# amathislab/HOISDF

Hardware: AMD Instinct MI355X
Metric: samples/sec (img + 2048 SDF queries) fwd+bwd at 1/2/4/8 MI355X (higher is better)
Workload: dtype f32 (emulated contractions, f32 accumulate, f16x2 form: operands as scaled hi + lo f16 pieces x 3 products - 22 operand bits, one power-of-two scale per ROW of a linear layer's row operand, per (sample, head) of the attention operands, per weight matrix; the attention backward's dS as three pieces x

## Files before the change

hoisdf_amd/csrc/chain.h:

```cpp
#pragma once
#include <stdlib.h>

#include <mutex>
#include <unordered_map>

#include "common.h"

namespace hoisdf {
namespace {

constexpr long EMU_MIN_ROWS = 2048;
constexpr long EMU_DW_MIN_ROWS = 8192;

inline bool al16(const void* p) { return (reinterpret_cast<uintptr_t>(p) & 15) == 0; }

struct SavedMags {
  std::mutex mu;
  std::unordered_map<const void*, int> on;
  void put(const void* key, bool v) { if (!key) return; std::lock_guard<std::mutex> l(mu); if (on.size() > 8192) on.clear(); on[key] = v ? 1 : 0; }
  int get(const void* key) { std::lock_guard<std::mutex> l(mu); auto it = on.find(key); return it == on.end() ? -1 : it->second; }
};
inline SavedMags& saved_mags() { static SavedMags s; return s; }

struct Ctx {
  hipStream_t st; void* stream;
  Bump* ws;
  bool dry;
  bool emu;
  int rc = HOISDF_OK;
  bool ok() const { return rc == HOISDF_OK; }
};

inline bool emu_small(const Ctx& c, long M, const float* a, long lda, const float* W, long ldw, int N, int K) {
  if (!c.emu || M > hoisdf_linear_emu_small_max_rows() || N % 4 || K % 4 || lda % 4 || ldw % 4) return false;
  return c.dry || hoisdf_linear_emu_small_supported(a, lda, W, ldw, M, N, K);
}
bool emu_rows(const Ctx& c, long M, const float* a, long lda, int contraction) {
  return c.emu && M >= EMU_MIN_ROWS && contraction % 4 == 0 && lda % 4 == 0 && (c.dry || al16(a));
}
const void* image_of(Ctx& c, const void* given, const float* W, int ldw, int N, int K, int transpose) {
  if (given) return given;
  void* img = c.ws->take(hoisdf_linear_emu_image_bytes(transpose ? K : N, transpose ? N : K));
  if (c.dry) return nullptr;
  if (!img) { c.rc = HOISDF_ERR_WORKSPACE; return nullptr; }
  c.rc = hoisdf_linear_emu_prepare(W, ldw, N, K, transpose, img, c.stream);
  return img;
}
void lin_fwd(Ctx& c, const float* x, int ldx, const float* W, int ldw, const void* img, const float* b, float* y, int ldy, long M, int N,
             int K, int act, float p, uint64_t seed, uint32_t* bits, int K_pad = 0, const uint32_t* x_mag = nullptr, uint32_t* y_mag = nullptr,
             uint32_t* y_heads = nullptr, int head_L = 0) {
  if (!c.ok()) return;
  if (K_pad < K || (K_pad + 15) / 16 != (K + 15) / 16) K_pad = K;
  if (emu_rows(c, M, x, ldx, K_pad)) {
    const void* im = image_of(c, img, W, ldw, N, K, 0);
    if (c.dry || !c.ok()) return;
    c.rc = linear_fwd_emu_mag(x, ldx, im, b, y, ldy, M, N, K_pad, act, p, seed, bits, x_mag, y_mag, c.stream, y_heads, head_L);
    return;
  }
  if (c.dry) return;
  if (emu_small(c, M, x, ldx, W, ldw, N, K)) { c.rc = hoisdf_linear_fwd_emu_small(x, ldx, W, ldw, b, y, ldy, M, N, K, act, p, seed, bits, c.stream); return; }
  c.rc = hoisdf_linear_fwd(x, ldx, W, ldw, b, y, ldy, M, N, K, act, p, seed, bits, c.stream);
}
void lin_bwd_input(Ctx& c, const float* dy, int lddy, const uint32_t* bits, float p, const float* W, int ldw, const void* img_t, float* dx,
                   int lddx, long M, int N, int K, int accumulate, const uint32_t* dy_mag = nullptr, uint32_t* dx_mag = nullptr,
                   uint32_t* dx_heads = nullptr, int head_L = 0) {
  if (!c.ok()) return;
  if (!bits) p = 0.f;
  if (emu_rows(c, M, dy, lddy, N)) {
    const void* im = image_of(c, img_t, W, ldw, N, K, 1);
    if (c.dry || !c.ok()) return;
    c.rc = linear_bwd_input_emu_mag(dy, lddy, bits, p, im, dx, lddx, M, N, K, accumulate, dy_mag, accumulate ? nullptr : dx_mag, c.stream,
                                    accumulate ? nullptr : dx_heads, head_L);
    return;
  }
  if (c.dry) return;
  if (emu_small(c, M, dy, lddy, W, ldw, N, K)) { c.rc = hoisdf_linear_bwd_input_emu_small(dy, lddy, bits, p, W, ldw, dx, lddx, M, N, K, accumulate, c.stream); return; }
  c.rc = hoisdf_linear_bwd_input(dy, lddy, bits, p, W, ldw, dx, lddx, M, N, K, accumulate, c.stream);
}
void lin_bwd_weight(Ctx& c, const float* dy, int lddy, const uint32_t* bits, float p, const float* x, int ldx, float* dW, float* db, long M,
                    int N, int K, int K_pad = 0, const uint32_t* dy_mag = nullptr, const uint32_t* x_mag = nullptr) {
  if (!c.ok()) return;
  if (!bits) p = 0.f;
  if (K_pad < K) K_pad = K;
  const bool emu = c.emu && M >= EMU_DW_MIN_ROWS && (N < K ? N : K) >= 64 && N % 4 == 0 && K_pad % 4 == 0 && lddy % 4 == 0 && ldx % 4 == 0 &&
                   (c.dry || (al16(dy) && al16(x) && al16(dW)));
  if (emu) {
    const long nws = hoisdf_linear_bwd_weight_emu_workspace(M, N, K_pad);
    float* w = c.ws->floats(nws > 4 ? nws : 4);
    if (!c.dry) {
      if (!w) { c.rc = HOISDF_ERR_WORKSPACE; return; }
      if (dy_mag || x_mag) c.rc = linear_bwd_weight_emu_mag(dy, lddy, bits, p, x, ldx, dW, K_pad, db, M, N, K_pad, w, nws, dy_mag, x_mag, c.stream);
      else c.rc = hoisdf_linear_bwd_weight_emu(dy, lddy, bits, p, x, ldx, dW, K_pad, db, M, N, K_pad, w, nws, c.stream);
    }
    return;
  }
  if (c.emu && M <= hoisdf_linear_emu_small_max_rows()) {
    if (!c.dry) c.rc = hoisdf_linear_bwd_weight_emu_small(dy, lddy, bits, p, x, ldx, dW, K_pad, db, M, N, K_pad, c.stream);
    return;
  }
  long nws = 0; float* w = nullptr;
  if (deterministic_mode()) {
    nws = hoisdf_linear_bwd_weight_workspace(M, N, K_pad);
    if (nws > 0) w = c.ws->floats(nws);
    if (!c.dry && nws > 0 && !w) { c.rc = HOISDF_ERR_WORKSPACE; return; }
  }
  if (c.dry) return;
  c.rc = hoisdf_linear_bwd_weight(dy, lddy, bits, p, x, ldx, dW, K_pad, db, M, N, K_pad, w, nws, c.stream);
}


}
}
```

hoisdf_amd/csrc/heads.hip:

```cpp
#include "chain.h"

using namespace hoisdf;

namespace {
constexpr int MLP_MAX = HOISDF_MLP_MAX_LAYERS;
inline long bits_words(int N) { return (N + 31) / 32; }

struct MlpSaved { float* h[MLP_MAX]; uint32_t* bits[MLP_MAX]; uint32_t* mag; };

bool mlp_ok(const hoisdf_mlp* m) {
  if (!m || m->n_layers < 1 || m->n_layers > MLP_MAX) return false;
  for (int i = 0; i <= m->n_layers; ++i) if (m->dims[i] <= 0) return false;
  return true;
}
void mlp_carve(const hoisdf_mlp* m, long M, Bump& b, MlpSaved& s) {
  const int last = m->n_layers - 1;
  for (int i = 0; i < m->n_layers; ++i) {
    s.h[i] = i < last ? b.floats(M * m->dims[i + 1]) : nullptr;
    const bool act = i < last || m->act_last;
    s.bits[i] = act ? static_cast<uint32_t*>(b.take(M * bits_words(m->dims[i + 1]) * 4)) : nullptr;
  }
  s.mag = static_cast<uint32_t*>(b.take((long)m->n_layers * M * 4));
}
inline bool chain_mags_on(const Ctx& c, long M) { return c.emu && emu_form_h2() && M >= EMU_MIN_ROWS; }
uint32_t* chain_mags(Ctx& c, long M, int n) {
  if (!chain_mags_on(c, M)) return nullptr;
  uint32_t* p = static_cast<uint32_t*>(c.ws->take((long)n * M * 4));
  if (c.dry || !p || !c.ok()) return nullptr;
  if (hipMemsetAsync(p, 0, (size_t)n * M * 4, c.st) != hipSuccess) { c.rc = HOISDF_ERR_LAUNCH; return nullptr; }
  return p;
}
void mlp_forward(Ctx& c, const hoisdf_mlp* m, const float* x, int ldx, long M, const MlpSaved& s, float* y, int ldy, const uint32_t* x_mag = nullptr) {
  const int last = m->n_layers - 1;
  const float* in = x; int ldin = ldx;
  uint32_t* mg = chain_mags_on(c, M) && !c.dry && s.mag && c.ok() ? s.mag : nullptr;
  if (!c.dry) saved_mags().put(s.mag, mg != nullptr);
  if (mg && hipMemsetAsync(mg, 0, (size_t)m->n_layers * M * 4, c.st) != hipSuccess) { c.rc = HOISDF_ERR_LAUNCH; return; }
  const uint32_t* in_mag = mg ? x_mag : nullptr;
  if (mg && !in_mag && emu_rows(c, M, x, ldx, m->dims[0])) {
    if ((c.rc = emu_mag_measure(x, ldx, M, m->dims[0], mg, c.st)) != HOISDF_OK) return;
    in_mag = mg;
  }
  for (int i = 0; i < m->n_layers; ++i) {
    float* out = i < last ? s.h[i] : y;
    const int ldo = i < last ? m->dims[i + 1] : ldy;
    uint32_t* out_mag = mg && i < last && emu_rows(c, M, in, ldin, m->dims[i]) ? mg + (long)(i + 1) * M : nullptr;
    lin_fwd(c, in, ldin, m->w[i], m->dims[i], m->img[i], m->b[i], out, ldo, M, m->dims[i + 1], m->dims[i], s.bits[i] ? 1 : 0, 0.f, 0, s.bits[i], 0,
            in_mag, out_mag);
    in = out; ldin = ldo; in_mag = out_mag;
  }
}
void mlp_backward(Ctx& c, const hoisdf_mlp* m, const hoisdf_mlp_grads* G, const float* x, int ldx, long M, const MlpSaved& s, const float* dy,
                  int lddy, float* dx, int lddx, int accumulate_dx, const uint32_t* x_mag = nullptr) {
  const float* g = dy; int ldg = lddy;
  const int last = m->n_layers - 1;
  uint32_t* mg = chain_mags(c, M, m->n_layers + 1);
  const bool fwd_mags = mg && s.mag && saved_mags().get(s.mag) != 0;
  const uint32_t* g_mag = nullptr;
  if (mg && emu_rows(c, M, dy, lddy, m->dims[last + 1])) {
    if ((c.rc = emu_mag_measure(dy, lddy, M, m->dims[last + 1], mg + (long)(last + 1) * M, c.st)) != HOISDF_OK) return;
    g_mag = mg + (long)(last + 1) * M;
  }
  for (int i = last; i >= 0; --i) {
    const float* in = i > 0 ? s.h[i - 1] : x;
    const int ldin = i > 0 ? m->dims[i] : ldx;
    const uint32_t* in_mag = !fwd_mags ? nullptr : i > 0 ? (emu_rows(c, M, i > 1 ? s.h[i - 2] : x, i > 1 ? m->dims[i - 1] : ldx, m->dims[i - 1]) ? s.mag + (long)i * M : nullptr)
                                                         : (x_mag ? x_mag : (emu_rows(c, M, x, ldx, m->dims[0]) ? s.mag : nullptr));
    lin_bwd_weight(c, g, ldg, s.bits[i], 0.f, in, ldin, G->dw[i], G->db[i], M, m->dims[i + 1], m->dims[i], 0, g_mag, g_mag ? in_mag : nullptr);
    if (i == 0 && !dx) break;
    float* gin = i > 0 ? c.ws->floats(M * m->dims[i]) : dx;
    const int ldgin = i > 0 ? m->dims[i] : lddx;
    if (!c.dry && c.ok() && !gin) { c.rc = HOISDF_ERR_WORKSPACE; return; }
    uint32_t* gin_mag = mg && i > 0 && emu_rows(c, M, g, ldg, m->dims[i + 1]) ? mg + (long)i * M : nullptr;
    lin_bwd_input(c, g, ldg, s.bits[i], 0.f, m->w[i], m->dims[i], m->img_t[i], gin, ldgin, M, m->dims[i + 1], m->dims[i], i == 0 ? accumulate_dx : 0,
                  g_mag, gin_mag);
    g = gin; ldg = ldgin; g_mag = gin_mag;
  }
}
const uint32_t* enc_mag(const Ctx& c, const hoisdf_mlp* m, const float* x, int ldx, long M, const MlpSaved& s) {
  return chain_mags_on(c, M) && !c.dry && s.mag && saved_mags().get(s.mag) != 0 && emu_rows(c, M, x, ldx, m->dims[0]) ? s.mag : nullptr;
}
bool grads_ok(const hoisdf_mlp* m, const hoisdf_mlp_grads* G) {
  if (!G) return false;
  for (int i = 0; i < m->n_layers; ++i) if (!G->dw[i] || !G->db[i]) return false;
  return true;
}

struct TokSaved { float* feat; float* fea; MlpSaved mlp; };
void tok_carve(const hoisdf_mlp* m, long M, bool own_feat, Bump& b, TokSaved& s) {
  s.feat = own_feat ? b.floats(M * m->dims[0]) : nullptr;
  s.fea = b.floats(M * m->dims[m->n_layers]);
  mlp_carve(m, M, b, s.mlp);
}

struct VoteSaved { float *off, *cls, *stats; MlpSaved vote, cl; };
void vote_carve(const hoisdf_mlp* mv, const hoisdf_mlp* mc, long M, int LB, int J, Bump& b, VoteSaved& s) {
  s.off = b.floats(M * 3 * J); s.cls = b.floats(M * J); s.stats = b.floats((long)LB * J * 2);
  mlp_carve(mv, M, b, s.vote); mlp_carve(mc, M, b, s.cl);
}
}

extern "C" long hoisdf_tokens_saved_bytes(const hoisdf_mlp* mlp, long n_rows, int gather_inside) {
  if (!mlp_ok(mlp) || n_rows <= 0) return 0;
  Bump b(nullptr, 0); TokSaved s;
  tok_carve(mlp, n_rows, gather_inside != 0, b, s);
  return b.off + 256;
}

static int tokens_backward(const hoisdf_mlp* mlp, const hoisdf_mlp_grads* G, const float* feat, long M, TokSaved& s, const float* dtok,
                           const float* sdf, const float* beta, float* dfeat, int accumulate_dfeat, float* dbeta, int B, int P, int S, int row0,
                           int D, Bump& ws, bool dry, void* stream) {
  Ctx c{as_stream(stream), stream, &ws, dry, gemm_emu_mode()};
  const int F = mlp->dims[mlp->n_layers];
  float* dfea = ws.floats(M * F);
  float* part = ws.floats(hoisdf_token_build_bwd_partials());
  if (!dry) {
    if (!dfea || !part) { set_error("tokens_bwd: workspace too small"); return HOISDF_ERR_WORKSPACE; }
    c.rc = hoisdf_token_build_bwd_ordered(dtok, s.fea, F, sdf, beta, dfea, F, dbeta, part, B, P, S, row0, D, stream);
  }
  mlp_backward(c, mlp, G, feat, mlp->dims[0], M, s.mlp, dfea, F, dfeat, mlp->dims[0], accumulate_dfeat);
  if (c.ok() && !dry && ws.overflow) { set_error("tokens_bwd: workspace too small"); return HOISDF_ERR_WORKSPACE; }
  return c.rc;
}

extern "C" long hoisdf_tokens_workspace_bytes(const hoisdf_mlp* mlp, long n_rows, int backward_pass) {
  if (!mlp_ok(mlp) || n_rows <= 0) return 0;
  Bump ws(nullptr, 0), sv(nullptr, 0);
  TokSaved s; tok_carve(mlp, n_rows, false, sv, s);
  Ctx c{nullptr, nullptr, &ws, true, gemm_emu_mode()};
  if (backward_pass) {
    hoisdf_mlp_grads G{};
    (void)tokens_backward(mlp, &G, nullptr, n_rows, s, nullptr, nullptr, nullptr, reinterpret_cast<float*>(1), 0, nullptr, 1, 1, 1, 0, 1, ws, true, nullptr);
  } else {
    mlp_forward(c, mlp, nullptr, mlp->dims[0], n_rows, s.mlp, nullptr, mlp->dims[mlp->n_layers]);
  }
  return ws.off + 256;
}

extern "C" int hoisdf_tokens_fwd(const hoisdf_pyramid* pyr, const float* points, const float* center, const float* cam_intr, float scale,
                                 int img_h, int img_w, const float* feat_in, const float* cam_in, const hoisdf_mlp* mlp, const float* pe,
                                 const float* sdf, const float* beta_ptr, float* tok, float* fea_out, float* cam_out, int B, int P, int S,
                                 int row0, int D, void* saved, long saved_bytes, void* workspace, long workspace_bytes, void* stream) {
  HOISDF_REQUIRE(mlp_ok(mlp) && center && pe && sdf && beta_ptr && tok && saved && workspace, HOISDF_ERR_INVALID, "tokens_fwd: null pointer / bad MLP");
  HOISDF_REQUIRE(B > 0 && P > 0 && S >= row0 + P && row0 >= 0 && mlp->act_last && mlp->dims[mlp->n_layers] == D - 33, HOISDF_ERR_INVALID,
                 "tokens_fwd: bad sizes (the MLP must end in D - 33 = %d activated columns)", D - 33);
  const bool gather = feat_in == nullptr;
  HOISDF_REQUIRE(gather ? (pyr && points && cam_intr && cam_out) : (cam_in != nullptr), HOISDF_ERR_INVALID,
                 "tokens_fwd: either gathered rows + their camera points, or a pyramid + points + cam_out");
  const long M = (long)B * P;
  HOISDF_REQUIRE(saved_bytes >= hoisdf_tokens_saved_bytes(mlp, M, gather), HOISDF_ERR_WORKSPACE, "tokens_fwd: saved buffer of %ld bytes, need %ld", saved_bytes,
                 hoisdf_tokens_saved_bytes(mlp, M, gather));
// ... 9 lines not shown
  }
  mlp_forward(c, mlp, feat, C, M, s.mlp, s.fea, F);
  if (c.ok()) c.rc = hoisdf_token_build_fwd(cam, center, pe, s.fea, F, sdf, beta_ptr, tok, B, P, S, row0, D, stream);
  if (c.ok() && fea_out && hipMemcpyAsync(fea_out, s.fea, sizeof(float) * M * F, hipMemcpyDeviceToDevice, c.st) != hipSuccess) c.rc = HOISDF_ERR_LAUNCH;
  if (c.ok() && (sv.overflow || ws.overflow)) c.rc = HOISDF_ERR_WORKSPACE;
  if (c.rc == HOISDF_ERR_WORKSPACE) set_error("tokens_fwd: workspace (%ld bytes) too small", workspace_bytes);
  return c.rc;
}

extern "C" int hoisdf_tokens_bwd(const hoisdf_pyramid_grad* dpyr, const float* points, const float* center, const float* cam_intr, float scale,
                                 int img_h, int img_w, const float* feat_in, const hoisdf_mlp* mlp, const float* sdf, const float* beta_ptr,
                                 const float* dtok, const void* saved, long saved_bytes, const hoisdf_mlp_grads* grads, float* dfeat,
                                 int accumulate_dfeat, float* dbeta, int B, int P, int S, int row0, int D, void* workspace, long workspace_bytes,
                                 void* stream) {
  HOISDF_REQUIRE(mlp_ok(mlp) && grads_ok(mlp, grads) && sdf && beta_ptr && dtok && saved && dbeta && workspace, HOISDF_ERR_INVALID,
                 "tokens_bwd: null pointer (every weight-gradient buffer is required, zero-filled)");
  const bool gather = feat_in == nullptr;
  const long M = (long)B * P;
  HOISDF_REQUIRE(B > 0 && P > 0 && saved_bytes >= hoisdf_tokens_saved_bytes(mlp, M, gather), HOISDF_ERR_INVALID, "tokens_bwd: bad sizes / saved buffer");
  HOISDF_REQUIRE(gather ? (points && center && cam_intr) : true, HOISDF_ERR_INVALID, "tokens_bwd: the gather's arguments are needed again");
  Bump sv(const_cast<void*>(saved), saved_bytes), ws(workspace, workspace_bytes);
  TokSaved s; tok_carve(mlp, M, gather, sv, s);
  const int C = mlp->dims[0];
  float* df = dfeat;
  int acc = accumulate_dfeat;
  if (gather && dpyr && !df) {
    df = ws.floats(M * C); acc = 0;
    if (!df) { set_error("tokens_bwd: workspace too small"); return HOISDF_ERR_WORKSPACE; }
  }
  int rc = tokens_backward(mlp, grads, gather ? s.feat : feat_in, M, s, dtok, sdf, beta_ptr, df, acc, dbeta, B, P, S, row0, D, ws, false, stream);
  if (rc == HOISDF_OK && gather && dpyr && df)
    rc = hoisdf_project_gather_bwd(dpyr, points, nullptr, M, P, center, cam_intr, scale, img_h, img_w, df, C, stream);
  return rc;
}

extern "C" long hoisdf_heads_vote_saved_bytes(const hoisdf_mlp* vote, const hoisdf_mlp* cls, int L, int B, int P, int J) {
  if (!mlp_ok(vote) || !mlp_ok(cls) || L <= 0 || B <= 0 || P <= 0 || J <= 0) return 0;
  Bump b(nullptr, 0); VoteSaved s;
  vote_carve(vote, cls, (long)L * B * P, L * B, J, b, s);
  return b.off + 256;
}

static int heads_vote_backward(const hoisdf_mlp* mv, const hoisdf_mlp* mc, const hoisdf_mlp_grads* Gv, const hoisdf_mlp_grads* Gc, const float* enc,
                               const float* pts, const float* gt, float radius, const float* joints, VoteSaved& s, const float* djoints,
                               const float* dl3d, const float* dbce, float* denc, int L, int B, int P, int J, Bump& ws, bool dry, void* stream) {
  Ctx c{as_stream(stream), stream, &ws, dry, gemm_emu_mode()};
  const long M = (long)L * B * P;
  float* doff = ws.floats(M * 3 * J); float* dcls = ws.floats(M * J);
  if (!dry) {
    if (!doff || !dcls) { set_error("heads_vote_bwd: workspace too small"); return HOISDF_ERR_WORKSPACE; }
    c.rc = hoisdf_vote_loss_bwd(s.off, s.cls, pts, gt, radius, joints, s.stats, djoints, dl3d, dbce, doff, dcls, L, B, P, J, stream);
  }
  const int E = mv->dims[0];
  mlp_backward(c, mv, Gv, enc, E, M, s.vote, doff, 3 * J, denc, E, 0);
  mlp_backward(c, mc, Gc, enc, E, M, s.cl, dcls, J, denc, E, 1, enc_mag(c, mv, enc, E, M, s.vote));
  if (c.ok() && !dry && ws.overflow) { set_error("heads_vote_bwd: workspace too small"); return HOISDF_ERR_WORKSPACE; }
  return c.rc;
}

extern "C" long hoisdf_heads_vote_workspace_bytes(const hoisdf_mlp* vote, const hoisdf_mlp* cls, int L, int B, int P, int J, int backward_pass) {
  if (!mlp_ok(vote) || !mlp_ok(cls) || L <= 0 || B <= 0 || P <= 0 || J <= 0) return 0;
  const long M = (long)L * B * P;
  Bump ws(nullptr, 0), sv(nullptr, 0);
  VoteSaved s; vote_carve(vote, cls, M, L * B, J, sv, s);
  if (backward_pass) {
    hoisdf_mlp_grads G{};
    (void)heads_vote_backward(vote, cls, &G, &G, nullptr, nullptr, nullptr, 0.f, nullptr, s, nullptr, nullptr, nullptr, reinterpret_cast<float*>(1), L, B, P, J, ws,
                              true, nullptr);
  } else {
    Ctx c{nullptr, nullptr, &ws, true, gemm_emu_mode()};
    mlp_forward(c, vote, nullptr, vote->dims[0], M, s.vote, nullptr, 3 * J);
    mlp_forward(c, cls, nullptr, cls->dims[0], M, s.cl, nullptr, J);
  }
  return ws.off + 256;
}

extern "C" int hoisdf_heads_vote_fwd(const float* enc, const hoisdf_mlp* vote, const hoisdf_mlp* cls, const float* pts, const float* joint_gt_mm,
                                     float radius, float* joints, float* l3d_sum, float* bce_sum, float* near_sum, int L, int B, int P, int J,
                                     void* saved, long saved_bytes, void* workspace, long workspace_bytes, void* stream) {
  HOISDF_REQUIRE(enc && mlp_ok(vote) && mlp_ok(cls) && pts && joint_gt_mm && joints && l3d_sum && bce_sum && near_sum && saved && workspace,
                 HOISDF_ERR_INVALID, "heads_vote_fwd: null pointer / bad MLP");
  HOISDF_REQUIRE(L > 0 && B > 0 && P > 0 && J > 0 && vote->dims[vote->n_layers] == 3 * J && cls->dims[cls->n_layers] == J &&
                     vote->dims[0] == cls->dims[0] && !vote->act_last && !cls->act_last,
                 HOISDF_ERR_INVALID, "heads_vote_fwd: the vote MLP must end in 3 J = %d, the class MLP in J = %d plain columns", 3 * J, J);
  HOISDF_REQUIRE(saved_bytes >= hoisdf_heads_vote_saved_bytes(vote, cls, L, B, P, J), HOISDF_ERR_WORKSPACE, "heads_vote_fwd: saved buffer too small");
  const long M = (long)L * B * P;
  Bump sv(saved, saved_bytes), ws(workspace, workspace_bytes);
  VoteSaved s; vote_carve(vote, cls, M, L * B, J, sv, s);
  Ctx c{as_stream(stream), stream, &ws, false, gemm_emu_mode()};
  const int E = vote->dims[0];
  mlp_forward(c, vote, enc, E, M, s.vote, s.off, 3 * J);
  mlp_forward(c, cls, enc, E, M, s.cl, s.cls, J, enc_mag(c, vote, enc, E, M, s.vote));
  if (c.ok()) c.rc = hoisdf_vote_loss_fwd(s.off, s.cls, pts, joint_gt_mm, radius, joints, s.stats, l3d_sum, bce_sum, near_sum, L, B, P, J, stream);
  if (c.ok() && (sv.overflow || ws.overflow)) c.rc = HOISDF_ERR_WORKSPACE;
  if (c.rc == HOISDF_ERR_WORKSPACE) set_error("heads_vote_fwd: workspace (%ld bytes) too small", workspace_bytes);
  return c.rc;
}

extern "C" int hoisdf_heads_vote_bwd(const float* enc, const hoisdf_mlp* vote, const hoisdf_mlp* cls, const float* pts, const float* joint_gt_mm,
                                     float radius, const float* joints, const void* saved, long saved_bytes, const float* djoints,
                                     const float* dl3d_sum, const float* dbce_sum, const hoisdf_mlp_grads* vote_grads,
                                     const hoisdf_mlp_grads* cls_grads, float* denc, int L, int B, int P, int J, void* workspace,
                                     long workspace_bytes, void* stream) {
  HOISDF_REQUIRE(enc && mlp_ok(vote) && mlp_ok(cls) && grads_ok(vote, vote_grads) && grads_ok(cls, cls_grads) && pts && joint_gt_mm && joints && saved &&
                     denc && workspace,
                 HOISDF_ERR_INVALID, "heads_vote_bwd: null pointer (every weight-gradient buffer is required, zero-filled)");
  HOISDF_REQUIRE(L > 0 && B > 0 && P > 0 && J > 0 && saved_bytes >= hoisdf_heads_vote_saved_bytes(vote, cls, L, B, P, J), HOISDF_ERR_INVALID,
                 "heads_vote_bwd: bad sizes / saved buffer");
  Bump sv(const_cast<void*>(saved), saved_bytes), ws(workspace, workspace_bytes);
  VoteSaved s; vote_carve(vote, cls, (long)L * B * P, L * B, J, sv, s);
  return heads_vote_backward(vote, cls, vote_grads, cls_grads, enc, pts, joint_gt_mm, radius, joints, s, djoints, dl3d_sum, dbce_sum, denc, L, B, P, J, ws, false,
                             stream);
}
```

hoisdf_amd/csrc/sdf_query.hip:

```cpp
#include "common.h"

using namespace hoisdf;

namespace {
constexpr int HID0 = 512, LAT = 256, PF = 33, H1 = 223, X0 = LAT + PF, CAT_K = 516, X0_COL = 224;
constexpr int CAT_LD = 544;
inline long align64(long v) { return (v + 63) / 64 * 64; }
constexpr long EMU_MIN_ROWS_Q = 2048;

inline long emu_scratch_bytes(int C) {
  const long a = hoisdf_linear_emu_image_bytes(HID0, C), b = hoisdf_linear_emu_image_bytes(HID0, CAT_K);
  return ((a > b ? a : b) + 255) / 256 * 256;
}

int layer(const float* x, int ldx, const float* W, int ldw, const float* b, float* y, int ldy, long M, int N, int K,
          int K_pad, float drop_p, uint64_t seed, void* emu_img, const void* given, void* stream, const uint32_t* x_mag = nullptr,
          uint32_t* y_mag = nullptr, bool* y_has = nullptr) {
  if (y_has) *y_has = false;
  if (emu_img && M >= EMU_MIN_ROWS_Q && hoisdf_linear_emu_supported(x, ldx, K_pad) && (K_pad + 15) / 16 == (K + 15) / 16) {
    if (!given) { if (int rc = hoisdf_linear_emu_prepare(W, ldw, N, K, 0, emu_img, stream)) return rc; }
    if (y_has) *y_has = y_mag != nullptr;
    return linear_fwd_emu_mag(x, ldx, given ? given : emu_img, b, y, ldy, M, N, K_pad, 1, drop_p, seed, nullptr, x_mag, y_mag, stream);
  }
  return hoisdf_linear_fwd(x, ldx, W, ldw, b, y, ldy, M, N, K, 1, drop_p, seed, nullptr, stream);
// ... 157 lines not shown
  int rc = hoisdf_lattice_fill(center, cam_intr, bbox, scale, bins_n, B, offsets, pts, sidx, lidx, stream);
  if (rc) return rc;
  rc = hoisdf_sdf_query_fwd(pyr, pts, sidx, n, 1, center, cam_intr, scale, img_h, img_w, nullptr, nullptr, w, clamp, drop_p, seed, sdf, raw, pe,
                            nullptr, qws, qbytes, stream);
  if (rc) return rc;
  rc = hoisdf_select_smallest_abs(raw, offsets, counts_device, B, num_points, sel, stream);
  if (rc) return rc;
  const long ns = (long)B * num_points;
  rc = hoisdf_gather_rows(pts, 3, sel, ns, 3, points_out, 3, stream);
  if (rc) return rc;
  rc = hoisdf_gather_rows(sdf, 1, sel, ns, 1, sdf_out, 1, stream);
  if (rc) return rc;
  if (pe_out) rc = hoisdf_gather_rows(pe, 30, sel, ns, 30, pe_out, 30, stream);
  return rc;
}

#include "chain.h"

namespace {
struct TrainSaved { float *feat, *ha, *cat, *h0, *h2, *h3, *raw; uint32_t *ba, *bf, *b0, *b1, *b2, *b3; uint32_t* mag; };
enum { TM_FEAT = 0, TM_HA = 1, TM_CAT = 2, TM_H0 = 3, TM_H2 = 4, TM_N = 5 };
inline bool train_mags(const Ctx& c, long n) { return c.emu && emu_form_h2() && n >= EMU_MIN_ROWS; }
inline long bits_words(int N) { return (N + 31) / 32; }
void train_carve(long n, int C, Bump& b, TrainSaved& s) {
  s.feat = b.floats(n * C); s.ha = b.floats(n * HID0); s.cat = b.floats(n * CAT_LD); s.h0 = b.floats(n * HID0); s.h2 = b.floats(n * HID0);
  s.h3 = b.floats(n * HID0); s.raw = b.floats(n);
  s.ba = static_cast<uint32_t*>(b.take(n * bits_words(HID0) * 4)); s.bf = static_cast<uint32_t*>(b.take(n * bits_words(LAT) * 4));
  s.b0 = static_cast<uint32_t*>(b.take(n * bits_words(HID0) * 4)); s.b1 = static_cast<uint32_t*>(b.take(n * bits_words(H1 + 1) * 4));
  s.b2 = static_cast<uint32_t*>(b.take(n * bits_words(HID0) * 4)); s.b3 = static_cast<uint32_t*>(b.take(n * bits_words(HID0) * 4));
  s.mag = static_cast<uint32_t*>(b.take((long)TM_N * n * 4));
}
}

extern "C" long hoisdf_sdf_query_train_saved_bytes(long n_rows, int C) {
  if (n_rows <= 0 || C <= 0) return 0;
  Bump b(nullptr, 0); TrainSaved s;
  train_carve(n_rows, C, b, s);
  return b.off + 256;
}

static int sdf_train_forward(const hoisdf_pyramid* pyr, const float* points, const int32_t* sample_idx, long n, int rps, const float* center,
                             const float* cam_intr, float scale, int img_h, int img_w, const hoisdf_sdf_weights* w, float clamp, float drop_p,
                             uint64_t seed, float* sdf, float* pe, float* cam_out, Bump& saved, Bump& ws, bool dry, void* stream) {
  Ctx c{as_stream(stream), stream, &ws, dry, gemm_emu_mode()};
  TrainSaved s;
  const int C = w ? w->C : 1;
  train_carve(n, C, saved, s);
  const bool mags = train_mags(c, n) && !dry && s.mag;
  if (!dry) saved_mags().put(s.mag, mags);
  auto mg = [&](int i) -> uint32_t* { return mags ? s.mag + (long)i * n : nullptr; };
  if (!dry) {
    if (mags) c.rc = hipMemsetAsync(s.mag, 0, (size_t)TM_N * n * 4, c.st) == hipSuccess ? HOISDF_OK : HOISDF_ERR_LAUNCH;
    if (c.ok()) c.rc = project_gather_fwd_mag(pyr, points, sample_idx, n, rps, center, cam_intr, scale, img_h, img_w, s.feat, C, cam_out, nullptr, mg(TM_FEAT), stream);
    if (c.ok()) c.rc = hipMemsetAsync(s.cat, 0, sizeof(float) * n * CAT_LD, c.st) == hipSuccess ? HOISDF_OK : HOISDF_ERR_LAUNCH;
  }
  float* x0 = dry ? nullptr : s.cat + X0_COL;
  lin_fwd(c, s.feat, C, w->sdfin_w0, C, w->emu_img[0], w->sdfin_b0, s.ha, HID0, n, HID0, C, 1, 0.f, 0, s.ba, 0, mg(TM_FEAT), mg(TM_HA));
  lin_fwd(c, s.ha, HID0, w->sdfin_w1, HID0, w->emu_img[1], w->sdfin_b1, x0, CAT_LD, n, LAT, HID0, 1, 0.f, 0, s.bf, 0, mg(TM_HA), mg(TM_CAT));
  if (!dry && c.ok()) c.rc = posenc_fwd_mag(points, n, s.cat, CAT_LD, X0_COL + LAT, pe, mg(TM_CAT), stream);
  lin_fwd(c, x0, CAT_LD, w->dec_w0, w->dec_ld0, w->emu_img[2], w->dec_b0, s.h0, HID0, n, HID0, X0, 1, drop_p, seed, s.b0, X0 + 3, mg(TM_CAT), mg(TM_H0));
  lin_fwd(c, s.h0, HID0, w->dec_w1, HID0, w->emu_img[3], w->dec_b1, s.cat, CAT_LD, n, H1 + 1, HID0, 1, drop_p, seed + 1, s.b1, 0, mg(TM_H0), mg(TM_CAT));
  lin_fwd(c, s.cat, CAT_LD, w->dec_w2, CAT_K, w->emu_img[4], w->dec_b2, s.h2, HID0, n, HID0, CAT_K, 1, drop_p, seed + 2, s.b2, 0, mg(TM_CAT), mg(TM_H2));
  lin_fwd(c, s.h2, HID0, w->dec_w3, HID0, w->emu_img[5], w->dec_b3, s.h3, HID0, n, HID0, HID0, 1, drop_p, seed + 3, s.b3, 0, mg(TM_H2), nullptr);
  if (!dry && c.ok()) c.rc = hoisdf_sdf_head_fwd(s.h3, HID0, w->dec_w4, w->dec_b4, s.raw, sdf, n, HID0, clamp, stream);
  return c.rc;
}

static int sdf_train_backward(const hoisdf_pyramid_grad* dpyr, const float* points, const int32_t* sample_idx, long n, int rps, const float* center,
                              const float* cam_intr, float scale, int img_h, int img_w, const hoisdf_sdf_weights* w, float clamp, float drop_p,
                              const float* d_sdf, const hoisdf_sdf_weight_grads* G, Bump& saved, Bump& ws, bool dry, void* stream) {
  Ctx c{as_stream(stream), stream, &ws, dry, gemm_emu_mode()};
  TrainSaved s;
  const int C = w ? w->C : 1;
  train_carve(n, C, saved, s);
  float* dh3 = ws.floats(n * HID0); float* dh2 = ws.floats(n * HID0); float* dcat = ws.floats(n * CAT_LD); float* dh0 = ws.floats(n * HID0);
  float* dha = ws.floats(n * HID0); float* dfeat = ws.floats(n * (long)C);
  if (!dry && (!dh3 || !dh2 || !dcat || !dh0 || !dha || !dfeat)) { set_error("sdf_query_bwd: workspace too small"); return HOISDF_ERR_WORKSPACE; }
  enum { BM_DH3 = 0, BM_DH2 = 1, BM_DCAT = 2, BM_DH0 = 3, BM_DHA = 4, BM_N = 5 };
  uint32_t* bmag = static_cast<uint32_t*>(ws.take((long)BM_N * n * 4));
  const bool mags = train_mags(c, n) && !dry && bmag && s.mag;
  const bool fmags = mags && saved_mags().get(s.mag) != 0;
  auto mg = [&](int i) -> uint32_t* { return mags ? bmag + (long)i * n : nullptr; };
  auto fm = [&](int i) -> const uint32_t* { return fmags ? s.mag + (long)i * n : nullptr; };
  if (mags) c.rc = hipMemsetAsync(bmag, 0, (size_t)BM_N * n * 4, c.st) == hipSuccess ? HOISDF_OK : HOISDF_ERR_LAUNCH;
  if (!dry && c.ok()) c.rc = sdf_head_bwd_mag(d_sdf, s.raw, s.h3, HID0, w->dec_w4, dh3, HID0, G->d_dec_w4, G->d_dec_b4, n, HID0, clamp, mg(BM_DH3), stream);
  lin_bwd_input(c, dh3, HID0, s.b3, drop_p, w->dec_w3, HID0, w->emu_img_t[5], dh2, HID0, n, HID0, HID0, 0, mg(BM_DH3), mg(BM_DH2));
  lin_bwd_weight(c, dh3, HID0, s.b3, drop_p, s.h2, HID0, G->d_dec_w3, G->d_dec_b3, n, HID0, HID0, 0, mg(BM_DH3), fm(TM_H2));
  lin_bwd_input(c, dh2, HID0, s.b2, drop_p, w->dec_w2, CAT_K, w->emu_img_t[4], dcat, CAT_LD, n, HID0, CAT_K, 0, mg(BM_DH2), mg(BM_DCAT));
  lin_bwd_weight(c, dh2, HID0, s.b2, drop_p, s.cat, CAT_LD, G->d_dec_w2, G->d_dec_b2, n, HID0, CAT_K, 0, mg(BM_DH2), fm(TM_CAT));
  lin_bwd_input(c, dcat, CAT_LD, s.b1, drop_p, w->dec_w1, HID0, w->emu_img_t[3], dh0, HID0, n, H1 + 1, HID0, 0, mg(BM_DCAT), mg(BM_DH0));
  lin_bwd_weight(c, dcat, CAT_LD, s.b1, drop_p, s.h0, HID0, G->d_dec_w1, G->d_dec_b1, n, H1 + 1, HID0, 0, mg(BM_DCAT), fm(TM_H0));
  float* dx0 = dry ? nullptr : dcat + X0_COL;
  const float* x0 = dry ? nullptr : s.cat + X0_COL;
  lin_bwd_input(c, dh0, HID0, s.b0, drop_p, w->dec_w0, w->dec_ld0, w->emu_img_t[2], dx0, CAT_LD, n, HID0, X0, 1, mg(BM_DH0), nullptr);
  lin_bwd_weight(c, dh0, HID0, s.b0, drop_p, x0, CAT_LD, G->d_dec_w0, G->d_dec_b0, n, HID0, X0, X0 + 3, mg(BM_DH0), fm(TM_CAT));
  lin_bwd_input(c, dx0, CAT_LD, s.bf, 0.f, w->sdfin_w1, HID0, w->emu_img_t[1], dha, HID0, n, LAT, HID0, 0, nullptr, mg(BM_DHA));
  lin_bwd_weight(c, dx0, CAT_LD, s.bf, 0.f, s.ha, HID0, G->d_sdfin_w1, G->d_sdfin_b1, n, LAT, HID0, 0, nullptr, fm(TM_HA));
  lin_bwd_input(c, dha, HID0, s.ba, 0.f, w->sdfin_w0, C, w->emu_img_t[0], dfeat, C, n, HID0, C, 0, mg(BM_DHA), nullptr);
  lin_bwd_weight(c, dha, HID0, s.ba, 0.f, s.feat, C, G->d_sdfin_w0, G->d_sdfin_b0, n, HID0, C, 0, mg(BM_DHA), fm(TM_FEAT));
  if (!dry && c.ok() && dpyr)
    c.rc = hoisdf_project_gather_bwd(dpyr, points, sample_idx, n, rps, center, cam_intr, scale, img_h, img_w, dfeat, C, stream);
  if (c.ok() && !dry && ws.overflow) { set_error("sdf_query_bwd: workspace too small"); return HOISDF_ERR_WORKSPACE; }
  return c.rc;
}

extern "C" long hoisdf_sdf_query_train_workspace_bytes(long n_rows, int C, int backward_pass) {
  if (n_rows <= 0 || C <= 0) return 0;
// ... 42 lines not shown
```

hoisdf_amd/ops.py:

```python
from __future__ import annotations

import ctypes as C
import math
import os
from typing import Optional, Sequence

import numpy as np
import torch

from . import _lib
from ._lib import (MLP_MAX_LAYERS, DecoderLayerDesc, DecoderLayerGrads, DecoderLayerWeights, EncoderLayerDesc,
                   EncoderLayerGrads, EncoderLayerWeights, Mlp, MlpGrads, PoseOutputs, Pyramid, SdfWeightGrads, SdfWeights, call, lib)
from .emu_images import WeightImageCache, prepare_batch_table

_SEED = [0x9E3779B97F4A7C15, 0]
_WEIGHT_GEN = [0]


def deterministic() -> bool:
    return bool(lib().hoisdf_get_deterministic())


def set_deterministic(on: bool) -> None:
    lib().hoisdf_set_deterministic(int(bool(on)))
# ... 184 lines not shown
        return (None, *out)


class _ProjectGather(torch.autograd.Function):
    @staticmethod
    def forward(ctx, points, sample_idx, center, cam_intr, scale, img_hw, acc, *levels):
        ctx.acc = acc
        pyr = PyramidNHWC(levels)
        pts = points.reshape(-1, 3).contiguous()
        _chk(pts, center, cam_intr)
        n = pts.shape[0]
        rps = points.shape[-2] if sample_idx is None else 1
        feat = torch.empty(n, pyr.C, device=pts.device, dtype=torch.float32)
        cam = torch.empty(n, 3, device=pts.device, dtype=torch.float32)
        s = pyr.struct()
        call("hoisdf_project_gather_fwd", C.byref(s), _p(pts), _p(sample_idx), n, rps, _p(center), _p(cam_intr),
             float(scale), img_hw[0], img_hw[1], _p(feat), pyr.C, _p(cam), None, _st())
        ctx.save_for_backward(pts, sample_idx, center, cam_intr)
        ctx.meta = (float(scale), img_hw, rps, [tuple(l.shape) for l in pyr.levels], pyr.B)
        ctx.mark_non_differentiable(cam)
        return feat, cam

    @staticmethod
    def backward(ctx, dfeat, _dcam):
        pts, sample_idx, center, cam_intr = ctx.saved_tensors
        scale, img_hw, rps, shapes, B = ctx.meta
        dfeat = dfeat.contiguous()
        acc = ctx.acc
        if acc is not None:
            grads = acc.bufs
            acc.flat.record_stream(torch.cuda.current_stream(dfeat.device))
        else:
            grads = [torch.zeros(sh, device=dfeat.device, dtype=torch.float32) for sh in shapes]
        g = _pyramid_struct(grads, B)
        call("hoisdf_project_gather_bwd", C.byref(g), _p(pts), _p(sample_idx), pts.shape[0], rps, _p(center),
             _p(cam_intr), scale, img_hw[0], img_hw[1], _p(dfeat), dfeat.shape[1], _st())
        if acc is not None:
            ev = torch.cuda.Event()
            ev.record(torch.cuda.current_stream(dfeat.device))
            acc.events.append(ev)
            acc.touched = True
            return (None,) * (7 + len(shapes))
        return (None, None, None, None, None, None, None, *grads)


def project_gather(pyr: PyramidNHWC, points, center, cam_intr, scale, img_hw=(256, 256), sample_idx=None):
    return _ProjectGather.apply(points, sample_idx, center.contiguous(), cam_intr.contiguous(), scale,
                                tuple(img_hw), pyr.acc, *pyr.levels)


_GEMM_EMU = os.environ.get("HOISDF_GEMM", "emu") != "f32"
_GEMM_EMU_MIN_ROWS = 2048
_GEMM_EMU_DW_MIN_ROWS = 8192
_GEMM_EMU_DW_MIN_WIDTH = 64
_EMU_CACHE = WeightImageCache()


def set_gemm_emu(on: bool) -> None:
    global _GEMM_EMU
    _GEMM_EMU = bool(on)
    lib().hoisdf_set_gemm_emu(int(_GEMM_EMU))


def gemm_emu() -> bool:
    return _GEMM_EMU


_EMU_SMALL_MAX = [None]


def _emu_small_max_rows() -> int:
    if _EMU_SMALL_MAX[0] is None:
        _EMU_SMALL_MAX[0] = lib().hoisdf_linear_emu_small_max_rows()
    return _EMU_SMALL_MAX[0]


def _emu_small_ok(M: int, a: torch.Tensor, lda: int, W: torch.Tensor, N: int, K: int) -> bool:
    if not _GEMM_EMU:
        return False
    return (1 <= M <= _emu_small_max_rows() and N % 4 == 0 and K % 4 == 0 and lda % 4 == 0 and W.stride(0) % 4 == 0
            and a.data_ptr() % 16 == 0 and W.data_ptr() % 16 == 0)


def _emu_ok(M: int, a: torch.Tensor, lda: int, contraction: int) -> bool:
    return (_GEMM_EMU and M >= _GEMM_EMU_MIN_ROWS and contraction % 4 == 0 and lda % 4 == 0
            and a.data_ptr() % 16 == 0)


def _emu_image(W: torch.Tensor, transpose: bool) -> torch.Tensor:
    return _EMU_CACHE.get(W, transpose, _WEIGHT_GEN[0])


_H2 = [None]


def _h2() -> bool:
    if _H2[0] is None:
        _H2[0] = lib().hoisdf_linear_emu_pieces() == 2
    return _H2[0]


def _mag_measure(a2, lda, M, K):
    if not _h2():
        return None
    words = torch.empty(max(int(M), 1), device=a2.device, dtype=torch.int32)
    call("hoisdf_mag_measure", _p(a2), lda, M, K, _p(words), _st())
    a2._hoisdf_words = (words, a2._version, a2.data_ptr(), lda, M, K)
    return words


def _head_measure(a2, lda, M, groups, L):
    nb = (M + L - 1) // L
    words = torch.empty(groups * nb, device=a2.device, dtype=torch.int32)
    call("hoisdf_head_mag_measure", _p(a2), lda, M, groups, L, _p(words), _st())
    return words


def _mag_known(a2, lda, M, K):
    t = getattr(a2, "_hoisdf_words", None)
    if t is not None and t[1:] == (a2._version, a2.data_ptr(), lda, M, K):
        return t[0]
    return None


def _gemm_fwd(x2, ldx, W, b, y, ldy, M, N, K, act, drop_p, seed, bits, x_mag=None, y_mag=None):
    if _emu_ok(M, x2, ldx, K):
        if _h2():
            if x_mag is None:
                x_mag = _mag_measure(x2, ldx, M, K)
            call("hoisdf_linear_fwd_emu_mag", _p(x2), ldx, _p(_emu_image(W, False)), _p(b), _p(y), ldy, M, N, K, int(act),
                 float(drop_p), seed, _p(bits), _p(x_mag), _p(y_mag), _st())
            return x_mag
        call("hoisdf_linear_fwd_emu", _p(x2), ldx, _p(_emu_image(W, False)), _p(b), _p(y), ldy, M, N, K, int(act),
             float(drop_p), seed, _p(bits), _st())
        return None
    call("hoisdf_linear_fwd_emu_small" if _emu_small_ok(M, x2, ldx, W, N, K) else "hoisdf_linear_fwd", _p(x2), ldx, _p(W), W.stride(0),
         _p(b), _p(y), ldy, M, N, K, int(act), float(drop_p), seed, _p(bits), _st())
    return None


def _gemm_bwd_input(dy2, lddy, bits, p, W, dx, lddx, M, N, K, accumulate, dy_mag=None):
    if _emu_ok(M, dy2, lddy, N):
        if _h2():
            if dy_mag is None:
                dy_mag = _mag_measure(dy2, lddy, M, N)
            call("hoisdf_linear_bwd_input_emu_mag", _p(dy2), lddy, _p(bits), float(p), _p(_emu_image(W, True)), _p(dx), lddx, M, N, K,
                 int(accumulate), _p(dy_mag), None, _st())
            return dy_mag
        call("hoisdf_linear_bwd_input_emu", _p(dy2), lddy, _p(bits), float(p), _p(_emu_image(W, True)), _p(dx), lddx, M, N, K,
             int(accumulate), _st())
        return None
    call("hoisdf_linear_bwd_input_emu_small" if _emu_small_ok(M, dy2, lddy, W, N, K) else "hoisdf_linear_bwd_input", _p(dy2), lddy,
         _p(bits), float(p), _p(W), W.stride(0), _p(dx), lddx, M, N, K, int(accumulate), _st())
    return None


def _gemm_bwd_weight(dy2, lddy, bits, p, x2, ldx, dW, db, M, N, K, x_mag=None, dy_mag=None, form=None):
    if _h2() and form != "b3":
        x_mag = x_mag if x_mag is not None else _mag_known(x2, ldx, M, K)
        dy_mag = dy_mag if dy_mag is not None else _mag_known(dy2, lddy, M, N)
    if (_GEMM_EMU and M >= _GEMM_EMU_DW_MIN_ROWS and min(N, K) >= _GEMM_EMU_DW_MIN_WIDTH and N % 4 == 0 and K % 4 == 0
            and lddy % 4 == 0 and ldx % 4 == 0 and dW.stride(0) == K and dy2.data_ptr() % 16 == 0 and x2.data_ptr() % 16 == 0
            and dW.data_ptr() % 16 == 0):
        nws = lib().hoisdf_linear_bwd_weight_emu_workspace(M, N, K)
        ws = torch.empty(max(nws, 4), device=dW.device, dtype=torch.float32)
        if form == "h2" or dy_mag is not None or x_mag is not None:
            call("hoisdf_linear_bwd_weight_emu_mag", _p(dy2), lddy, _p(bits), float(p), _p(x2), ldx, _p(dW), K, _p(db), M, N, K,
                 _p(ws), nws, _p(dy_mag), _p(x_mag), _st())
        else:
            call("hoisdf_linear_bwd_weight_emu", _p(dy2), lddy, _p(bits), float(p), _p(x2), ldx, _p(dW), K, _p(db), M, N, K,
                 _p(ws), nws, _st())
        return
    if M == 0:
        return
    if _GEMM_EMU and M <= _emu_small_max_rows():
        call("hoisdf_linear_bwd_weight_emu_small", _p(dy2), lddy, _p(bits), float(p), _p(x2), ldx, _p(dW), dW.stride(0), _p(db), M, N, K,
             _st())
        return
    ws, nws = None, 0
    if deterministic():
        nws = lib().hoisdf_linear_bwd_weight_workspace(M, N, K)
        ws = torch.empty(max(nws, 1), device=dW.device, dtype=torch.float32) if nws > 0 else None
    call("hoisdf_linear_bwd_weight", _p(dy2), lddy, _p(bits), float(p), _p(x2), ldx, _p(dW), dW.stride(0), _p(db), M, N, K,
         _p(ws), nws, _st())


class _Linear(torch.autograd.Function):
    @staticmethod
    def forward(ctx, x, W, b, act, drop_p, seed):
        x2 = _rows(x)
        W = W if W.stride(-1) == 1 else W.contiguous()
        _chk(x2, W, b)
        M, K = x2.shape
        N = W.shape[0]
        assert W.shape[1] == K, (W.shape, K)
        if drop_p > 0 and not act:
            raise RuntimeError("dropout without relu is not supported by linear()")
        y = torch.empty(M, N, device=x.device, dtype=torch.float32)
        need_bits = bool(act) and (x.requires_grad or W.requires_grad or (b is not None and b.requires_grad))
        bits = torch.empty(M, (N + 31) // 32, device=x.device, dtype=torch.int32) if need_bits else None
        ctx.x_mag = _gemm_fwd(x2, x2.stride(0) if M > 1 else K, W, b, y, N, M, N, K, act, drop_p, seed, bits)
        ctx.save_for_backward(x2, W, bits)
        ctx.meta = (int(act), float(drop_p), b is not None, x.shape)
        return y.view(*x.shape[:-1], N)

    @staticmethod
    def backward(ctx, dy):
        x2, W, bits = ctx.saved_tensors
        act, drop_p, has_b, xshape = ctx.meta
        M, K = x2.shape
        N = W.shape[0]
        dy2 = _rows(dy)
        lddy = dy2.stride(0) if M > 1 else N
        p = drop_p if bits is not None else 0.0
# ... 2178 lines not shown
```

Measured before the change: 445.7.

## Route narrow weight-grad GEMMs to emulated kernel and merge magnitude memsets

Lets the weight-gradient path use the emulated mag kernel when N is below 64, provided magnitude data is available, instead of falling back to the slower f32 path. The vote and cls heads now share one magnitude buffer, zeroed by a single memset in forward and backward rather than one per MLP. The zeroing memset of the SDF concat buffer is dropped. Dropping that memset risks reading stale padding columns if the later writes do not fully cover the buffer, and the dry-run path for narrow cases now carves workspace for both routes.

```diff
diff --git a/hoisdf_amd/csrc/chain.h b/hoisdf_amd/csrc/chain.h
--- a/hoisdf_amd/csrc/chain.h
+++ b/hoisdf_amd/csrc/chain.h
@@ -11,6 +11,7 @@
 
 constexpr long EMU_MIN_ROWS = 2048;
 constexpr long EMU_DW_MIN_ROWS = 8192;
+constexpr int EMU_DW_MIN_K = 64;
 
 inline bool al16(const void* p) { return (reinterpret_cast<uintptr_t>(p) & 15) == 0; }
 
@@ -82,7 +83,9 @@
   if (!c.ok()) return;
   if (!bits) p = 0.f;
   if (K_pad < K) K_pad = K;
-  const bool emu = c.emu && M >= EMU_DW_MIN_ROWS && (N < K ? N : K) >= 64 && N % 4 == 0 && K_pad % 4 == 0 && lddy % 4 == 0 && ldx % 4 == 0 &&
+  const bool narrow = N < EMU_DW_MIN_K;
+  const bool narrow_ok = !narrow || (emu_form_h2() && (c.dry || dy_mag || x_mag));
+  const bool emu = c.emu && M >= EMU_DW_MIN_ROWS && K_pad >= EMU_DW_MIN_K && narrow_ok && N % 4 == 0 && K_pad % 4 == 0 && lddy % 4 == 0 && ldx % 4 == 0 &&
                    (c.dry || (al16(dy) && al16(x) && al16(dW)));
   if (emu) {
     const long nws = hoisdf_linear_bwd_weight_emu_workspace(M, N, K_pad);
@@ -92,7 +95,7 @@
       if (dy_mag || x_mag) c.rc = linear_bwd_weight_emu_mag(dy, lddy, bits, p, x, ldx, dW, K_pad, db, M, N, K_pad, w, nws, dy_mag, x_mag, c.stream);
       else c.rc = hoisdf_linear_bwd_weight_emu(dy, lddy, bits, p, x, ldx, dW, K_pad, db, M, N, K_pad, w, nws, c.stream);
     }
-    return;
+    if (!(c.dry && narrow)) return;
   }
   if (c.emu && M <= hoisdf_linear_emu_small_max_rows()) {
     if (!c.dry) c.rc = hoisdf_linear_bwd_weight_emu_small(dy, lddy, bits, p, x, ldx, dW, K_pad, db, M, N, K_pad, c.stream);
diff --git a/hoisdf_amd/csrc/heads.hip b/hoisdf_amd/csrc/heads.hip
--- a/hoisdf_amd/csrc/heads.hip
+++ b/hoisdf_amd/csrc/heads.hip
@@ -13,14 +13,18 @@
   for (int i = 0; i <= m->n_layers; ++i) if (m->dims[i] <= 0) return false;
   return true;
 }
-void mlp_carve(const hoisdf_mlp* m, long M, Bump& b, MlpSaved& s) {
+void mlp_carve(const hoisdf_mlp* m, long M, Bump& b, MlpSaved& s, bool with_mag = true) {
   const int last = m->n_layers - 1;
   for (int i = 0; i < m->n_layers; ++i) {
     s.h[i] = i < last ? b.floats(M * m->dims[i + 1]) : nullptr;
     const bool act = i < last || m->act_last;
     s.bits[i] = act ? static_cast<uint32_t*>(b.take(M * bits_words(m->dims[i + 1]) * 4)) : nullptr;
   }
-  s.mag = static_cast<uint32_t*>(b.take((long)m->n_layers * M * 4));
+  s.mag = with_mag ? static_cast<uint32_t*>(b.take((long)m->n_layers * M * 4)) : nullptr;
+}
+void mags_carve(const hoisdf_mlp* ma, const hoisdf_mlp* mb, long M, Bump& b, MlpSaved& sa, MlpSaved& sb) {
+  sa.mag = static_cast<uint32_t*>(b.take((long)(ma->n_layers + mb->n_layers) * M * 4));
+  sb.mag = sa.mag ? sa.mag + (long)ma->n_layers * M : nullptr;
 }
 inline bool chain_mags_on(const Ctx& c, long M) { return c.emu && emu_form_h2() && M >= EMU_MIN_ROWS; }
 uint32_t* chain_mags(Ctx& c, long M, int n) {
@@ -30,12 +34,13 @@
   if (hipMemsetAsync(p, 0, (size_t)n * M * 4, c.st) != hipSuccess) { c.rc = HOISDF_ERR_LAUNCH; return nullptr; }
   return p;
 }
-void mlp_forward(Ctx& c, const hoisdf_mlp* m, const float* x, int ldx, long M, const MlpSaved& s, float* y, int ldy, const uint32_t* x_mag = nullptr) {
+void mlp_forward(Ctx& c, const hoisdf_mlp* m, const float* x, int ldx, long M, const MlpSaved& s, float* y, int ldy, const uint32_t* x_mag = nullptr,
+                 bool zero_mag = true) {
   const int last = m->n_layers - 1;
   const float* in = x; int ldin = ldx;
   uint32_t* mg = chain_mags_on(c, M) && !c.dry && s.mag && c.ok() ? s.mag : nullptr;
   if (!c.dry) saved_mags().put(s.mag, mg != nullptr);
-  if (mg && hipMemsetAsync(mg, 0, (size_t)m->n_layers * M * 4, c.st) != hipSuccess) { c.rc = HOISDF_ERR_LAUNCH; return; }
+  if (mg && zero_mag && hipMemsetAsync(mg, 0, (size_t)m->n_layers * M * 4, c.st) != hipSuccess) { c.rc = HOISDF_ERR_LAUNCH; return; }
   const uint32_t* in_mag = mg ? x_mag : nullptr;
   if (mg && !in_mag && emu_rows(c, M, x, ldx, m->dims[0])) {
     if ((c.rc = emu_mag_measure(x, ldx, M, m->dims[0], mg, c.st)) != HOISDF_OK) return;
@@ -51,10 +56,10 @@
   }
 }
 void mlp_backward(Ctx& c, const hoisdf_mlp* m, const hoisdf_mlp_grads* G, const float* x, int ldx, long M, const MlpSaved& s, const float* dy,
-                  int lddy, float* dx, int lddx, int accumulate_dx, const uint32_t* x_mag = nullptr) {
+                  int lddy, float* dx, int lddx, int accumulate_dx, const uint32_t* x_mag = nullptr, bool own_mags = true, uint32_t* mags = nullptr) {
   const float* g = dy; int ldg = lddy;
   const int last = m->n_layers - 1;
-  uint32_t* mg = chain_mags(c, M, m->n_layers + 1);
+  uint32_t* mg = own_mags ? chain_mags(c, M, m->n_layers + 1) : mags;
   const bool fwd_mags = mg && s.mag && saved_mags().get(s.mag) != 0;
   const uint32_t* g_mag = nullptr;
   if (mg && emu_rows(c, M, dy, lddy, m->dims[last + 1])) {
@@ -96,7 +101,8 @@
 struct VoteSaved { float *off, *cls, *stats; MlpSaved vote, cl; };
 void vote_carve(const hoisdf_mlp* mv, const hoisdf_mlp* mc, long M, int LB, int J, Bump& b, VoteSaved& s) {
   s.off = b.floats(M * 3 * J); s.cls = b.floats(M * J); s.stats = b.floats((long)LB * J * 2);
-  mlp_carve(mv, M, b, s.vote); mlp_carve(mc, M, b, s.cl);
+  mlp_carve(mv, M, b, s.vote, false); mlp_carve(mc, M, b, s.cl, false);
+  mags_carve(mv, mc, M, b, s.vote, s.cl);
 }
 }
 
@@ -212,8 +218,9 @@
     c.rc = hoisdf_vote_loss_bwd(s.off, s.cls, pts, gt, radius, joints, s.stats, djoints, dl3d, dbce, doff, dcls, L, B, P, J, stream);
   }
   const int E = mv->dims[0];
-  mlp_backward(c, mv, Gv, enc, E, M, s.vote, doff, 3 * J, denc, E, 0);
-  mlp_backward(c, mc, Gc, enc, E, M, s.cl, dcls, J, denc, E, 1, enc_mag(c, mv, enc, E, M, s.vote));
+  uint32_t* mg = chain_mags(c, M, mv->n_layers + 1 + mc->n_layers + 1);
+  mlp_backward(c, mv, Gv, enc, E, M, s.vote, doff, 3 * J, denc, E, 0, nullptr, false, mg);
+  mlp_backward(c, mc, Gc, enc, E, M, s.cl, dcls, J, denc, E, 1, enc_mag(c, mv, enc, E, M, s.vote), false, mg ? mg + (long)(mv->n_layers + 1) * M : nullptr);
   if (c.ok() && !dry && ws.overflow) { set_error("heads_vote_bwd: workspace too small"); return HOISDF_ERR_WORKSPACE; }
   return c.rc;
 }
@@ -249,8 +256,10 @@
   VoteSaved s; vote_carve(vote, cls, M, L * B, J, sv, s);
   Ctx c{as_stream(stream), stream, &ws, false, gemm_emu_mode()};
   const int E = vote->dims[0];
-  mlp_forward(c, vote, enc, E, M, s.vote, s.off, 3 * J);
-  mlp_forward(c, cls, enc, E, M, s.cl, s.cls, J, enc_mag(c, vote, enc, E, M, s.vote));
+  if (chain_mags_on(c, M) && s.vote.mag &&
+      hipMemsetAsync(s.vote.mag, 0, (size_t)(vote->n_layers + cls->n_layers) * M * 4, c.st) != hipSuccess) c.rc = HOISDF_ERR_LAUNCH;
+  if (c.ok()) mlp_forward(c, vote, enc, E, M, s.vote, s.off, 3 * J, nullptr, false);
+  if (c.ok()) mlp_forward(c, cls, enc, E, M, s.cl, s.cls, J, enc_mag(c, vote, enc, E, M, s.vote), false);
   if (c.ok()) c.rc = hoisdf_vote_loss_fwd(s.off, s.cls, pts, joint_gt_mm, radius, joints, s.stats, l3d_sum, bce_sum, near_sum, L, B, P, J, stream);
   if (c.ok() && (sv.overflow || ws.overflow)) c.rc = HOISDF_ERR_WORKSPACE;
   if (c.rc == HOISDF_ERR_WORKSPACE) set_error("heads_vote_fwd: workspace (%ld bytes) too small", workspace_bytes);
diff --git a/hoisdf_amd/csrc/sdf_query.hip b/hoisdf_amd/csrc/sdf_query.hip
--- a/hoisdf_amd/csrc/sdf_query.hip
+++ b/hoisdf_amd/csrc/sdf_query.hip
@@ -233,7 +233,6 @@
   if (!dry) {
     if (mags) c.rc = hipMemsetAsync(s.mag, 0, (size_t)TM_N * n * 4, c.st) == hipSuccess ? HOISDF_OK : HOISDF_ERR_LAUNCH;
     if (c.ok()) c.rc = project_gather_fwd_mag(pyr, points, sample_idx, n, rps, center, cam_intr, scale, img_h, img_w, s.feat, C, cam_out, nullptr, mg(TM_FEAT), stream);
-    if (c.ok()) c.rc = hipMemsetAsync(s.cat, 0, sizeof(float) * n * CAT_LD, c.st) == hipSuccess ? HOISDF_OK : HOISDF_ERR_LAUNCH;
   }
   float* x0 = dry ? nullptr : s.cat + X0_COL;
   lin_fwd(c, s.feat, C, w->sdfin_w0, C, w->emu_img[0], w->sdfin_b0, s.ha, HID0, n, HID0, C, 1, 0.f, 0, s.ba, 0, mg(TM_FEAT), mg(TM_HA));
diff --git a/hoisdf_amd/ops.py b/hoisdf_amd/ops.py
--- a/hoisdf_amd/ops.py
+++ b/hoisdf_amd/ops.py
@@ -260,7 +260,7 @@
 _GEMM_EMU = os.environ.get("HOISDF_GEMM", "emu") != "f32"
 _GEMM_EMU_MIN_ROWS = 2048
 _GEMM_EMU_DW_MIN_ROWS = 8192
-_GEMM_EMU_DW_MIN_WIDTH = 64
+_GEMM_EMU_DW_MIN_K = 64
 _EMU_CACHE = WeightImageCache()
 
 
@@ -367,7 +367,8 @@
     if _h2() and form != "b3":
         x_mag = x_mag if x_mag is not None else _mag_known(x2, ldx, M, K)
         dy_mag = dy_mag if dy_mag is not None else _mag_known(dy2, lddy, M, N)
-    if (_GEMM_EMU and M >= _GEMM_EMU_DW_MIN_ROWS and min(N, K) >= _GEMM_EMU_DW_MIN_WIDTH and N % 4 == 0 and K % 4 == 0
+    narrow_ok = N >= _GEMM_EMU_DW_MIN_K or (_h2() and form != "b3" and (form == "h2" or dy_mag is not None or x_mag is not None))
+    if (_GEMM_EMU and M >= _GEMM_EMU_DW_MIN_ROWS and K >= _GEMM_EMU_DW_MIN_K and narrow_ok and N % 4 == 0 and K % 4 == 0
             and lddy % 4 == 0 and ldx % 4 == 0 and dW.stride(0) == K and dy2.data_ptr() % 16 == 0 and x2.data_ptr() % 16 == 0
             and dW.data_ptr() % 16 == 0):
         nws = lib().hoisdf_linear_bwd_weight_emu_workspace(M, N, K)
```

After: 446.9, median of 3. No clear change (+0.3%).
